# multiplefish/VPLines-SLAM

Hardware: AMD Instinct MI355X
Metric: sliding-window BA solves/sec (10 KF, 200 pts + 80 lines, 5 iters) (higher is better)
Workload: dtype f64

## Files before the change

### vplines-slam_amd/csrc/ba_common.h

```cpp
#pragma once
#include <hip/hip_runtime.h>
#include "ba_types.h"
#include "vpl_math.h"

namespace vpl {

#ifdef VPL_STAMPS
#define VPL_STAMP(B, w, i) do { if (threadIdx.x == 0) (B).dbg[(size_t)(w) * 64 + (i)] = (long long)__builtin_readcyclecounter(); } while (0)
#define VPL_IVAL(acc) long long acc = 0
#define VPL_IVAL_START(t) long long t = __builtin_readcyclecounter()
#define VPL_IVAL_ADD(acc, t) acc += __builtin_readcyclecounter() - (t)
#define VPL_IVAL_LAP(acc, t) do { const long long now_ = __builtin_readcyclecounter(); acc += now_ - (t); t = now_; } while (0)
#define VPL_IVAL_STORE(cond, dst, ...) do { long long* dst_ = (dst); if (dst_ && (cond)) { const long long v_[] = {__VA_ARGS__}; \
  for (int i_ = 0; i_ < (int)(sizeof(v_) / sizeof(v_[0])); ++i_) dst_[i_] = v_[i_]; } } while (0)
#else
#define VPL_STAMP(B, w, i) do {} while (0)
#define VPL_IVAL(acc) do {} while (0)
#define VPL_IVAL_START(t) do {} while (0)
#define VPL_IVAL_ADD(acc, t) do {} while (0)
#define VPL_IVAL_LAP(acc, t) do {} while (0)
#define VPL_IVAL_STORE(cond, dst, ...) do {} while (0)
#endif

__device__ __forceinline__ void count_active(const DevBatch& B, int k) {
  if (B.act && threadIdx.x == 0 && B.launch < ACT_SLOTS) atomicAdd(&B.act[4 * B.launch + k], 1);
}

__device__ __forceinline__ int ordered_window(const DevBatch& B) {
  const int w = B.ord_it == 0 ? (int)blockIdx.x : B.order[(size_t)(B.ord_it & 1) * B.nW + blockIdx.x];
  return __builtin_amdgcn_readfirstlane(w);
}

__device__ __forceinline__ double wave_sum(double v) {
#pragma unroll
  for (int o = 32; o > 0; o >>= 1) v += __shfl_xor(v, o, 64);
  return v;
}

template <int CTRL>
__device__ __forceinline__ double dpp_shr_f64(double v) {
  const int lo = __builtin_amdgcn_update_dpp(0, __double2loint(v), CTRL, 0xf, 0xf, true);
  const int hi = __builtin_amdgcn_update_dpp(0, __double2hiint(v), CTRL, 0xf, 0xf, true);
  return __hiloint2double(hi, lo);
}
__device__ __forceinline__ double row_sum16(double v) {
  v += dpp_shr_f64<0x111>(v);
  v += dpp_shr_f64<0x112>(v);
  v += dpp_shr_f64<0x114>(v);
  v += dpp_shr_f64<0x118>(v);
  return v;
}

__device__ __forceinline__ double wave_sum_dpp(double v) {
  v = row_sum16(v);
  double t = 0.0;
#pragma unroll
  for (int l = 15; l < 64; l += 16)
    t += __hiloint2double(__builtin_amdgcn_readlane(__double2hiint(v), l), __builtin_amdgcn_readlane(__double2loint(v), l));
  return t;
}

__device__ __forceinline__ double block_sum(double v, double* red) {
  const int lane = threadIdx.x & 63, wv = threadIdx.x >> 6, nw = (blockDim.x + 63) >> 6;
  v = wave_sum(v);
  __syncthreads();
  if (lane == 0) red[wv] = v;
  __syncthreads();
  if (threadIdx.x == 0) {
    double s = 0;
    for (int i = 0; i < nw; ++i) s += red[i];
    red[16] = s;
  }
  __syncthreads();
  return red[16];
}

__device__ __forceinline__ void lds_add(double* p, double v) { unsafeAtomicAdd(p, v); }

__host__ __device__ __forceinline__ int cam2vis(int c) {
  if (c >= 165) return 66 + (c - 165);
  int o = c % 15;
  return o < 6 ? 6 * (c / 15) + o : -1;
}

__device__ __forceinline__ void tri_decode(int idx, int& r, int& c) {
  int rr = (int)((sqrtf(8.0f * (float)idx + 1.0f) - 1.0f) * 0.5f);
  while ((rr + 1) * (rr + 2) / 2 <= idx) ++rr;
  while (rr * (rr + 1) / 2 > idx) --rr;
  r = rr;
  c = idx - rr * (rr + 1) / 2;
}

__device__ __forceinline__ PreInt load_preint(const DevPreint& d) {
  PreInt p;
  p.sum_dt = d.sum_dt;
  p.dp = V3{d.dp[0], d.dp[1], d.dp[2]};
  p.dv = V3{d.dv[0], d.dv[1], d.dv[2]};
  p.dq = Q4{d.dq[3], d.dq[0], d.dq[1], d.dq[2]};
  p.lba = V3{d.lba[0], d.lba[1], d.lba[2]};
  p.lbg = V3{d.lbg[0], d.lbg[1], d.lbg[2]};
#pragma unroll
  for (int k = 0; k < 9; ++k) {
    p.dp_dba.m[k] = d.dp_dba[k];
    p.dp_dbg.m[k] = d.dp_dbg[k];
    p.dq_dbg.m[k] = d.dq_dbg[k];
    p.dv_dba.m[k] = d.dv_dba[k];
    p.dv_dbg.m[k] = d.dv_dbg[k];
  }
  return p;
}

__device__ __forceinline__ void prior_block_dx(int kind, const double* x, const double* x0, double* dx) {
  if (kind == 1) {
#pragma unroll
    for (int k = 0; k < 9; ++k) dx[k] = x[k] - x0[k];
  } else {
    dx[0] = x[0] - x0[0]; dx[1] = x[1] - x0[1]; dx[2] = x[2] - x0[2];
    Q4 dq = qmul(qinv(qpose(x0)), qpose(x));
    double sgn = (dq.w >= 0) ? 2.0 : -2.0;
    dx[3] = sgn * dq.x; dx[4] = sgn * dq.y; dx[5] = sgn * dq.z;
  }
}

__device__ __forceinline__ double readlane_f64(double v, int srclane) {
  const int lo = __builtin_amdgcn_readlane(__double2loint(v), srclane);
  const int hi = __builtin_amdgcn_readlane(__double2hiint(v), srclane);
  return __hiloint2double(hi, lo);
}
template <int J>
__device__ __forceinline__ double swizzle_row_f64(double v) {
  const int lo = __builtin_amdgcn_mov_dpp(__double2loint(v), 0x150 + J, 0xf, 0xf, false);
  const int hi = __builtin_amdgcn_mov_dpp(__double2hiint(v), 0x150 + J, 0xf, 0xf, false);
  return __hiloint2double(hi, lo);
}

template <int J>
// ... 63 lines not shown
```

### vplines-slam_amd/csrc/ba_ctx.h

```cpp
#pragma once
#include <functional>
#include <map>
#include <string>

#include "vplines_ba.h"
#include "ba_types.h"
#include "ba_stage.h"
#include "ba_restore.h"

struct vpl_ctx {
  int device = 0;
  hipStream_t stream = nullptr;
  DevBatch B;
  std::vector<DevAlloc> allocs;
  bool guards = false;
  std::string err;
  int maxW = 0, maxP = 0, maxPO = 0, maxL = 0, maxLO = 0;
  int nW = 0;
  vpl_ba_options opt;
  bool upload_open = false;
  std::vector<int> h_nP, h_nL;
  std::vector<std::vector<int>> h_lmap;
  std::vector<int> h_mg_m;
  std::vector<int> h_mg_n;
  std::vector<int> h_mg_nb;
  std::vector<int> h_passthrough;
  std::vector<vpl_prior> h_pass_priors;
  bool any_second_new = false;
  int maxPriorN = 0;
  bool prior_resident = false;
  int prior_resident_nW = 0;
  std::vector<int> layout_key;
  bool layout_valid = false;
  bool force_general = false;
  bool schur_mostly_wide = false;
  bool schur_never_wide = false;
  bool schur_wide_all = false;
  bool step_fused = true;
  size_t marg_smem = 0;
  int marg_nmax = 0;
  bool marg_small = false;
  int prior_rule = VPL_PRIOR_PIVOTED_CHOLESKY;
  hipGraphExec_t graph_exec[3] = {nullptr, nullptr, nullptr};
  bool use_graph = true;
  int restore_pending = RESTORE_NONE;
  bool restore_fold = true;
  bool timing = false;
  std::map<std::string, std::pair<double, int>> ktimes;
  std::vector<std::pair<const char*, double>> ltimes;
  int* d_act = nullptr;
  std::vector<std::string> kname_store;
  bool leg_timing = false;
  hipEvent_t leg_ev[6] = {nullptr, nullptr, nullptr, nullptr, nullptr, nullptr};
  double odo_ms[3] = {0, 0, 0};
  std::function<int()> pending;
  Stage stage;
  size_t last_upload_bytes = 0;
  struct vpl_odo* odo = nullptr;
};

static void drop_graph(vpl_ctx* c) {
  for (hipGraphExec_t& g : c->graph_exec)
    if (g) { (void)hipGraphExecDestroy(g); g = nullptr; }
}

static int restore_states(vpl_ctx* c, int mode) {
  if (mode == RESTORE_NONE || c->nW < 1) return VPL_OK;
  const DevBatch& B = c->B;
  const size_t W = c->nW;
  HIPCHK(c, hipSetDevice(c->device));
  HIPCHK(c, hipMemcpyAsync(B.pose, B.pose_0, W * 77 * 8, hipMemcpyDeviceToDevice, c->stream));
  HIPCHK(c, hipMemcpyAsync(B.sb, B.sb_0, W * 99 * 8, hipMemcpyDeviceToDevice, c->stream));
  HIPCHK(c, hipMemcpyAsync(B.ex, B.ex_0, W * 7 * 8, hipMemcpyDeviceToDevice, c->stream));
  HIPCHK(c, hipMemcpyAsync(B.invd, B.invd_0, W * B.maxP * 8, hipMemcpyDeviceToDevice, c->stream));
  if (mode == RESTORE_LINES) HIPCHK(c, hipMemcpyAsync(B.plk, B.plk_0, W * B.maxL * 6 * 8, hipMemcpyDeviceToDevice, c->stream));
  return VPL_OK;
}
static int restore_event(vpl_ctx* c, RestoreEvent ev, int* prep = nullptr) {
  const RestoreStep s = restore_step(c->restore_pending, ev, c->restore_fold);
  c->restore_pending = s.pending;
  if (prep) *prep = s.prep;
  return restore_states(c, s.flush);
// ... 50 lines not shown
```

### vplines-slam_amd/csrc/ba_lin.h

```cpp
#pragma once
#include "ba_common.h"

namespace vpl {

typedef double v4d_lin __attribute__((ext_vector_type(4)));
constexpr int LIN_THREADS = 512;
constexpr int STG_LD = 17;
constexpr int LIN_STAGE = 8 * 32 * STG_LD;
constexpr int PRE_LDS = 62;
constexpr int LIN_HW = 720;
constexpr int PREP_NMAX = 112;
__host__ __device__ constexpr int lin_stage_doubles(int maxL) {
  const int ln = 8 * LIN_HW + 38 * maxL;
  const int pt = LIN_STAGE + 78 * 36 + NV;
  const int m = ln > pt ? ln : pt;
  return m > 4650 + 3570 ? m : 4650 + 3570;
}
constexpr int PREP_THREADS = 640;
inline size_t prep_smem(int max_prior_n) {
  const int ns = max_prior_n < PREP_NMAX ? max_prior_n : PREP_NMAX;
  return (size_t)((PREP_THREADS / 64) * 675 + ns * ns + ns + 84) * sizeof(double);
}
constexpr size_t PREP_SMEM = (size_t)((PREP_THREADS / 64) * 675 + PREP_NMAX * PREP_NMAX + PREP_NMAX + 84) * sizeof(double);

// ... 146 lines not shown
          acc = __builtin_amdgcn_mfma_f64_16x16x4f64(av, bv, acc, 0, 0, 0);
        }
        const double vals[4] = {acc.x, acc.y, acc.z, acc.w};
#pragma unroll
        for (int v = 0; v < 4; ++v) {
          const int r = 16 * ta + kk + 4 * v, c2 = cb;
          if (r < n && c2 < n && (ta != tb || r >= c2)) {
            H[(size_t)r * n + c2] = vals[v];
            H[(size_t)c2 * n + r] = vals[v];
          }
        }
      }
    } else
    for (int idx = tid; idx < n * n; idx += blockDim.x) {
      int a = idx / n, b = idx % n;
      double s = 0;
      for (int k = 0; k < n; ++k) s += Js[(size_t)k * n + a] * Js[(size_t)k * n + b];
      H[idx] = s;
    }
    for (int c2 = tid; c2 < n; c2 += blockDim.x) {
      double s = 0;
      if (fits) {
#pragma unroll 8
        for (int k = 0; k < n; ++k) s += Jl[k * n + c2] * r0s[k];
      } else {
        const double* r0g = B.pr_r0 + (size_t)w * MAXPN;
#pragma unroll 8
        for (int k = 0; k < n; ++k) s += J0[(size_t)k * n + c2] * r0g[k];
      }
      B.pr_g0[(size_t)w * MAXPN + c2] = s;
    }
    if (tid < B.pr_nb[w]) {
      int kind = B.pr_kind[(size_t)w * MAXPB + tid], fr = B.pr_frame[(size_t)w * MAXPB + tid];
      int idx = B.pr_idx[(size_t)w * MAXPB + tid];
      int base = kind == 0 ? 15 * fr : kind == 1 ? 15 * fr + 6 : 165;
      int ls = kind == 1 ? 9 : 6;
      for (int k = 0; k < ls; ++k) B.pr_map[(size_t)w * MAXPN + idx + k] = base + k;
    }
  }
  if (tid == 0) {
    TrState t;
    t.radius = 1e4; t.mu = 1e-8; t.x_cost = 0; t.cand_cost = 0; t.model_cost_change = 0; t.x_norm = 0;
    t.step_norm = 0; t.dogleg_step_norm = 0; t.alpha = 0; t.a1 = t.a2 = t.a3 = 0; t.initial_cost = 0;
    t.iter = 0; t.status = 0; t.reuse = 0; t.step_valid = 0; t.fresh_lin = 0; t.num_successful = 0; t.num_invalid = 0;
    t.pad = 0;
    B.tr[w] = t;
  }
}
__global__ __launch_bounds__(PREP_THREADS) void k_prep(DevBatch B, int nstage, int restore) {
  extern __shared__ double psm[];
  prep_body(B, blockIdx.x, psm, nstage, restore);
}

constexpr int HV_DOUBLES = 78 * 36;
constexpr int LIN_PART = 78 * 36 + 72 + 8;
__host__ __device__ __forceinline__ int hvi(int r, int c) {
  const int br = r / 6, bc = c / 6;
  return 36 * (br * (br + 1) / 2 + bc) + 6 * (r - 6 * br) + (c - 6 * bc);
}

inline void lin_asm_entry(int r, int c, int* out) {
  int hv = 0, im = 0;
  const int vr = cam2vis(r), vc = cam2vis(c);
  if (vr >= 0 && vc >= 0) hv = hvi(vr, vc) + 1;
  if (r < 165) {
    const int fr = r / 15, ar = r - 15 * fr, fc = c / 15, bc = c - 15 * fc;
    if (fc == fr) im = 120 * fr + ar * (ar + 1) / 2 + bc + 1;
    else if (fc == fr - 1) im = 11 * 120 + 225 * (fr - 1) + 15 * ar + bc + 1;
  }
  out[0] = hv | im << 16;
  out[1] = r | c << 8;
}


__device__ __forceinline__ double* lin_pt_stage(double* imuJ, int wvi) { return imuJ + wvi * (32 * STG_LD); }
__device__ __forceinline__ double* lin_Hv2(double* imuJ) { return imuJ + LIN_STAGE; }
__device__ __forceinline__ double* lin_ln_Hw(double* imuJ, int wvi) { return imuJ + wvi * LIN_HW; }
__device__ __forceinline__ double* lin_ln_acc(double* imuJ) { return imuJ + 8 * LIN_HW; }
__device__ __forceinline__ double* lin_imuH(double* imuJ) { return imuJ + 4650; }

struct PriorBlock {
  int kind = 0, fr = 0, idx = 0;
  double x0[9];
};
__device__ __forceinline__ void prior_block_request(const DevBatch& B, const int w, const int tid, const int nb, PriorBlock& b) {
  if (tid < nb) {
    b.kind = B.pr_kind[(size_t)w * MAXPB + tid]; b.fr = B.pr_frame[(size_t)w * MAXPB + tid]; b.idx = B.pr_idx[(size_t)w * MAXPB + tid];
#pragma unroll
    for (int k = 0; k < 9; ++k) b.x0[k] = B.pr_x0[((size_t)w * MAXPB + tid) * 9 + k];
  }
}
__device__ __forceinline__ void prior_block_dx_store(const PriorBlock& b, const int tid, const int nb, const double* xp, const double* xs,
                                                     double* prdx) {
  if (tid < nb) {
    const double* x = b.kind == 0 ? xp + 7 * b.fr : b.kind == 1 ? xs + 9 * b.fr : xp + 77;
    double dx[9];
    prior_block_dx(b.kind, x, b.x0, dx);
    const int ls = b.kind == 1 ? 9 : 6;
    for (int k = 0; k < ls; ++k) prdx[b.idx + k] = dx[k];
  }
}
constexpr int LIN_PJ = 6;
struct PriorRegs {
  int n = 0, nb = 0;
  PriorBlock blk;
  int pmap = -1;
  double j0[LIN_PJ], hv[LIN_PJ], r0 = 0.0, g0 = 0.0;
};
constexpr int LIN_ASM_PER_THREAD = (NCP + LIN_THREADS - 1) / LIN_THREADS;

template <int ROLE>
__device__ __forceinline__ void lin_stage(const DevBatch& B, const int w, double* sm, double* xp, double* xs, double* pacc, const int PST, double* plds,
                                             int* invmap, int* tick, PriorRegs& P) {
  constexpr bool DO_PTS = ROLE != 2, DO_REST = ROLE != 1;
  const int tid = threadIdx.x, T = LIN_THREADS;
  for (int i = tid; i < HV_DOUBLES + NV; i += T) sm[i] = 0.0;
  if (DO_PTS) for (int i = tid; i < 14 * PST; i += T) pacc[i] = 0.0;
  for (int i = tid; i < 84; i += T) xp[i] = i < 77 ? B.pose[(size_t)w * 77 + i] : B.ex[(size_t)w * 7 + (i - 77)];
  if (DO_REST) {
    for (int i = tid; i < 99; i += T) xs[i] = B.sb[(size_t)w * 99 + i];
    for (int i = tid; i < 10 * PRE_LDS; i += T) {
      const int f = i / PRE_LDS;
      plds[i] = ((const double*)&B.pre[(size_t)w * NF + f + 1])[i - PRE_LDS * f];
    }
  }
  for (int i = tid; i < NC; i += T) invmap[i] = -1;
  if (tid < 5) tick[tid] = 0;
  P.n = DO_REST ? B.pr_n[w] : 0; P.nb = P.n > 0 ? B.pr_nb[w] : 0;
  const int n = P.n;
  const int prow = tid >> 3, psub = tid & 7;
  prior_block_request(B, w, tid, P.nb, P.blk);
  if (tid < n) P.pmap = B.pr_map[(size_t)w * MAXPN + tid];
  {
    const double* J0 = B.pr_J0 + (size_t)w * B.prS;
    const double* Hp = B.pr_H + (size_t)w * B.prS;
#pragma unroll
    for (int q = 0; q < LIN_PJ; ++q) {
      const int c = psub + 8 * q;
      const bool in = prow < n && c < n;
      P.j0[q] = in ? J0[(size_t)prow * n + c] : 0.0;
      P.hv[q] = in ? Hp[(size_t)prow * n + c] : 0.0;
    }
    if (prow < n && psub == 0) { P.r0 = B.pr_r0[(size_t)w * MAXPN + prow]; P.g0 = B.pr_g0[(size_t)w * MAXPN + prow]; }
  }
}

__device__ __forceinline__ void lin_prior(const DevBatch& B, const int w, const double* xp, const double* xs, double* prdx, double* prr, double* prg,
                                             double* prH, const int PRH_N, int* invmap, const PriorRegs& P, double& cost) {
  const int tid = threadIdx.x, T = LIN_THREADS;
  const int n = P.n;
  const int prow = tid >> 3, psub = tid & 7;
  double r0r = P.r0, g0r = P.g0;
  if (n > 0) {
    prior_block_dx_store(P.blk, tid, P.nb, xp, xs, prdx);
    if (tid < n) invmap[P.pmap] = tid;
    for (int i = tid + T; i < n; i += T) invmap[B.pr_map[(size_t)w * MAXPN + i]] = i;
    __syncthreads();
    const double* J0 = B.pr_J0 + (size_t)w * B.prS;
    const double* Hp = B.pr_H + (size_t)w * B.prS;
    for (int r = prow; r < n; r += T >> 3) {
      const bool first = r == prow;
      double s = 0, sg = 0;
// ... 116 lines not shown
        Hv[hvi(66 + a, 6 * f + c2)] += v;
      } else {
        gv[6 * f + (q - 57)] += v;
      }
    } else if (e < 714) {
      int a, c2;
      tri_decode(e - 693, a, c2);
      Hv[hvi(66 + a, 66 + c2)] += v;
    } else {
      gv[66 + (e - 714)] += v;
    }
  }
}

template <int MODE>
__device__ __forceinline__ void lin_imu_raw(const DevBatch& B, const int w, const double* xp, const double* xs, const double* plds, double* imuJ, double* imur,
                                               int* imuact, double (&sa)[2][4]) {
  constexpr bool MARG = MODE != 0;
  constexpr bool PRIOR_ONLY = MODE == 2;
  const int tid = threadIdx.x, T = LIN_THREADS, lane = tid & 63;
  for (int i = tid; i < 4650; i += T) imuJ[i] = 0.0;
#pragma unroll
  for (int q = 0; q < 2; ++q) {
    const int f = (tid >> 6) + 8 * q;
    const double* S = B.pre[(size_t)w * NF + (f < 10 ? f : 0) + 1].sqrt_info;
#pragma unroll
    for (int ks = 0; ks < 4; ++ks) {
      const int k = 4 * ks + (lane >> 4), i = lane & 15;
      sa[q][ks] = (f < 10 && i < 15 && k < 15 && k >= i) ? S[i * 15 + k] : 0.0;
    }
  }
  __syncthreads();
  if ((tid & 63) < 10 && tid < 128) {
    const int f = tid & 63, j = f + 1;
    const DevPreint& dp = *(const DevPreint*)(plds + PRE_LDS * f);
    bool act = MARG ? (j == 1 && dp.sum_dt < 10.0) : !(dp.sum_dt > 10.0);
    if (PRIOR_ONLY) act = false;
    if (tid < 64) imuact[f] = act ? 1 : 0;
    if (act) {
      PreInt p = load_preint(dp);
      if (tid < 64) {
        imu_residual_raw(p, xp + 7 * (j - 1), xs + 9 * (j - 1), xp + 7 * j, xs + 9 * j, B.opt.g_norm, imur + 15 * f);
      } else {
        ImuJac JB = imu_jacobian_raw(p, xp + 7 * (j - 1), xs + 9 * (j - 1), xp + 7 * j, xs + 9 * j, B.opt.g_norm);
        imu_jac_dense(JB, imuJ + 450 * f);
      }
    }
  }
}
__device__ __forceinline__ void lin_asm_request(const DevBatch& B, int2 (&asmd)[LIN_ASM_PER_THREAD]) {
  const int tid = threadIdx.x, T = LIN_THREADS;
#pragma unroll
  for (int u = 0; u < LIN_ASM_PER_THREAD; ++u) {
    const int e = u * T + tid;
    asmd[u] = ((const int2*)B.asm_tab)[e < NCP ? e : 0];
  }
}
__device__ __forceinline__ void lin_imu_whiten(double* imuJ, double* imur, const int* imuact, const double (&sa)[2][4]) {
  const int tid = threadIdx.x, T = LIN_THREADS, lane = tid & 63;
  double* imuH = lin_imuH(imuJ);
  const int wvi = tid >> 6, m16 = lane & 15, kk = lane >> 4;
  v4d_lin cd[2] = {{0, 0, 0, 0}, {0, 0, 0, 0}};
  for (int i = tid; i < 120; i += T) imuH[i] = 0.0;
#pragma unroll
  for (int q = 0; q < 2; ++q) {
    const int f = wvi + 8 * q;
    if (f >= 10) break;
    double* J = imuJ + 450 * f;
    double* rr = imur + 15 * f;
    const bool on = imuact[f] != 0;
    v4d_lin jw[2] = {{0, 0, 0, 0}, {0, 0, 0, 0}};
#pragma unroll
    for (int ct = 0; ct < 2; ++ct) {
      const int c = 16 * ct + m16;
#pragma unroll
      for (int ks = 0; ks < 4; ++ks) {
        const int k = 4 * ks + kk;
        const double bv = k < 15 ? (c < 30 ? J[k * 30 + c] : (c == 30 ? rr[k] : 0.0)) : 0.0;
        jw[ct] = __builtin_amdgcn_mfma_f64_16x16x4f64(on ? sa[q][ks] : 0.0, bv, jw[ct], 0, 0, 0);
      }
    }
    __builtin_amdgcn_wave_barrier();
    if (on) {
#pragma unroll
      for (int ct = 0; ct < 2; ++ct) {
        const double vals[4] = {jw[ct].x, jw[ct].y, jw[ct].z, jw[ct].w};
        const int c = 16 * ct + m16;
#pragma unroll
        for (int v = 0; v < 4; ++v) {
          const int r = kk + 4 * v;
          if (r < 15) {
            if (c < 30) J[r * 30 + c] = vals[v];
            else if (c == 30) rr[r] = vals[v];
          }
        }
      }
    }
    __builtin_amdgcn_fence(__ATOMIC_RELEASE, "workgroup");
    __builtin_amdgcn_wave_barrier();
    __builtin_amdgcn_fence(__ATOMIC_ACQUIRE, "workgroup");
    v4d_lin c00 = {0, 0, 0, 0}, c10 = {0, 0, 0, 0}, c11 = {0, 0, 0, 0};
#pragma unroll
    for (int ks = 0; ks < 4; ++ks) {
      const int k = 4 * ks + kk;
      const double lo = k < 15 ? J[k * 30 + m16] : 0.0;
      const double hi = (k < 15 && m16 < 14) ? J[k * 30 + 16 + m16] : 0.0;
      c00 = __builtin_amdgcn_mfma_f64_16x16x4f64(lo, lo, c00, 0, 0, 0);
      c10 = __builtin_amdgcn_mfma_f64_16x16x4f64(hi, lo, c10, 0, 0, 0);
// ... 6 lines not shown
      for (int v = 0; v < 4; ++v) {
        const int i0 = kk + 4 * v, j0 = m16;
        if (i0 < 15 && j0 < 15) keep[v] = v00[v];
        const int i1 = 16 + kk + 4 * v;
        if (i1 < 30) {
          if (j0 < 15) imuH[11 * 120 + 225 * f + 15 * (i1 - 15) + j0] = v10[v];
          else imuH[120 * (f + 1) + (i1 - 15) * (i1 - 14) / 2 + 0] = v10[v];
          const int j1 = 16 + m16;
          if (j1 < 30 && j1 <= i1) imuH[120 * (f + 1) + (i1 - 15) * (i1 - 14) / 2 + (j1 - 15)] = v11[v];
        }
        if (i0 == 15) {
          if (j0 < 15) imuH[11 * 120 + 225 * f + j0] = v00[v];
          else imuH[120 * (f + 1)] = v00[v];
        }
      }
      cd[q] = v4d_lin{keep[0], keep[1], keep[2], keep[3]};
    }
  }
  __syncthreads();
#pragma unroll
  for (int q = 0; q < 2; ++q) {
    const int f = wvi + 8 * q;
    if (f >= 10) break;
    const double keep[4] = {cd[q].x, cd[q].y, cd[q].z, cd[q].w};
#pragma unroll
    for (int v = 0; v < 4; ++v) {
      const int i0 = kk + 4 * v, j0 = m16;
      if (i0 < 15 && j0 <= i0) imuH[120 * f + i0 * (i0 + 1) / 2 + j0] += keep[v];
    }
  }
}
__device__ __forceinline__ void lin_imu_cost(const double* imur, const int* imuact, double& cost) {
  const int tid = threadIdx.x;
  if (tid < 10 && imuact[tid]) {
    double s = 0;
    for (int k = 0; k < 15; ++k) s += imur[15 * tid + k] * imur[15 * tid + k];
    cost += 0.5 * s;
  }
}

__device__ __forceinline__ void lin_handover_in(const DevBatch& B, const int w, double* sm, double& cost) {
  const int tid = threadIdx.x, T = LIN_THREADS;
  if (tid == 0) {
    while (__hip_atomic_load(&B.lin_flag[w], __ATOMIC_RELAXED, __HIP_MEMORY_SCOPE_AGENT) != 1) __builtin_amdgcn_s_sleep(32);
    __hip_atomic_store(&B.lin_flag[w], 0, __ATOMIC_RELAXED, __HIP_MEMORY_SCOPE_AGENT);
  }
  __syncthreads();
  const double* part = B.lin_part + (size_t)w * LIN_PART;
  for (int i = tid; i < HV_DOUBLES + NV; i += T) sm[i] += __hip_atomic_load(&part[i], __ATOMIC_RELAXED, __HIP_MEMORY_SCOPE_AGENT);
  if (tid == 0) cost += __hip_atomic_load(&part[HV_DOUBLES + NV], __ATOMIC_RELAXED, __HIP_MEMORY_SCOPE_AGENT);
  __syncthreads();
}

__device__ __forceinline__ void lin_assemble(const DevBatch& B, const int w, const double* Hv, const double* gv, double* imuJ, const double* imur,
                                                const double* prg, const double* prH, const int PRH_N, const int* invmap,
                                                const int* imuact, const int n, const bool ex_free,
                                                const int2 (&asmd)[LIN_ASM_PER_THREAD]) {
  const int tid = threadIdx.x, T = LIN_THREADS;
  const double* const imuH = lin_imuH(imuJ);
  double* Hout = B.Hcc + (size_t)w * NCP;
  const double* pH = B.pr_H + (size_t)w * B.prS;
  VPL_STAMP(B, w, 26);
  const bool prior_lds = n > 0 && n <= PRH_N;
  {
#pragma unroll
    for (int u = 0; u < LIN_ASM_PER_THREAD; ++u) {
      const int e = u * T + tid;
      if (e >= NCP) continue;
      const int hv = asmd[u].x & 0xffff, im = asmd[u].x >> 16, r = asmd[u].y & 255, c = asmd[u].y >> 8;
      const double vh = Hv[hv ? hv - 1 : 0], vi = imuH[im ? im - 1 : 0];
      const int ir = prior_lds ? invmap[r] : -1, ic = prior_lds ? invmap[c] : -1;
      const bool hp = ir >= 0 && ic >= 0;
      const int hi_ = ic > ir ? ic : ir, lo_ = ic > ir ? ir : ic;
      const double vp = prH[hp ? hi_ * (hi_ + 1) / 2 + lo_ : 0];
      double v = hv ? vh : 0.0;
      v += im ? vi : 0.0;
      v += hp ? vp : 0.0;
      if (!ex_free && r >= 165) v = 0.0;
      Hout[e] = v;
    }
  }
  VPL_STAMP(B, w, 27);
  if (n > PRH_N) {
    __syncthreads();
    const int np = n * (n + 1) / 2;
    for (int base = 0; base < np; base += 4 * T) {
      double ph[4];
      int tr_[4], tc_[4];
#pragma unroll
      for (int u = 0; u < 4; ++u) {
        const int e = base + u * T + tid;
        ph[u] = 0.0; tr_[u] = -1; tc_[u] = 0;
        if (e < np) {
          int i, j;
          tri_decode(e, i, j);
          ph[u] = pH[(size_t)i * n + j];
          const int ri = B.pr_map[(size_t)w * MAXPN + i], rj = B.pr_map[(size_t)w * MAXPN + j];
          tr_[u] = ri > rj ? ri : rj;
          tc_[u] = ri > rj ? rj : ri;
        }
      }
#pragma unroll
      for (int u = 0; u < 4; ++u)
        if (tr_[u] >= 0 && (ex_free || tr_[u] < 165)) Hout[(size_t)tr_[u] * (tr_[u] + 1) / 2 + tc_[u]] += ph[u];
    }
  }
  for (int r = tid; r < NC; r += T) {
    double v = 0.0;
    const int vr = cam2vis(r);
    if (vr >= 0) v += gv[vr];
    if (r < 165) {
      const int fr = r / 15;
      if (fr >= 1 && imuact[fr - 1]) {
        const double* J = imuJ + 450 * (fr - 1);
        const double* rr = imur + 15 * (fr - 1);
        const int a = r - 15 * (fr - 1);
        double s = 0;
#pragma unroll
        for (int k = 0; k < 15; ++k) s += J[k * 30 + a] * rr[k];
        v += s;
      }
      if (fr < 10 && imuact[fr]) {
        const double* J = imuJ + 450 * fr;
        const double* rr = imur + 15 * fr;
        const int a = r - 15 * fr;
        double s = 0;
#pragma unroll
        for (int k = 0; k < 15; ++k) s += J[k * 30 + a] * rr[k];
        v += s;
      }
    }
    if (n > 0 && invmap[r] >= 0) v += prg[invmap[r]];
// ... 437 lines not shown
```

### vplines-slam_amd/csrc/ba_upload.h

```cpp
#pragma once
#include "ba_ctx.h"
#include "ba_odo.h"
#include "ba_pack.h"
#include "host_common.h"

static void to_dev_preint(const vpl_preintegration& p, DevPreint& d) {
  d.sum_dt = p.sum_dt;
  for (int k = 0; k < 3; ++k) { d.dp[k] = p.delta_p[k]; d.dv[k] = p.delta_v[k]; d.lba[k] = p.linearized_ba[k]; d.lbg[k] = p.linearized_bg[k]; }
  for (int k = 0; k < 4; ++k) d.dq[k] = p.delta_q[k];
  auto blk = [&](double* o, int r0, int c0) {
    for (int i = 0; i < 3; ++i)
      for (int j = 0; j < 3; ++j) o[3 * i + j] = p.jacobian[(r0 + i) * 15 + c0 + j];
  };
  blk(d.dp_dba, 0, 9); blk(d.dp_dbg, 0, 12); blk(d.dq_dbg, 3, 12); blk(d.dv_dba, 6, 9); blk(d.dv_dbg, 6, 12);
  std::memcpy(d.cov, p.covariance, sizeof(d.cov));
  std::memset(d.sqrt_info, 0, sizeof(d.sqrt_info));
}

struct UploadArena {
  Span<double> pose, sb, ex, invd, plk, pt_obs, ln_obs, fail_ref, orth, pr_x0, pr_r0;
  Span<int> nP, nL, pt_start, pt_nobs, pt_off, ln_start, ln_nobs, ln_off, ln_tri, pu_cnt, pu_cnt0, sk_tab, sk_wave, path, nLO, lo_ln,
      ll_tab, ll_np, ps_list, ps_cnt, orth_in, pr_n, pr_nb, pr_kind, pr_frame, pr_idx, mg_n, mg_nb, mg_kind, mg_frame, mg_idx, mg_cam, mg_m;
  Span<DevPreint> pre;
  std::vector<Span<double>> J0;
// ... 424 lines not shown
  B.opt.marginalization_flag = opt->marginalization_flag;
  B.opt.remove_line_outliers = opt->remove_line_outliers;
  B.opt.sqrt_info_point = opt->focal_length / 1.5;
  B.opt.sqrt_info_line = opt->line_factor;
  B.opt.sqrt_info_vp = opt->vp_factor;
  B.opt.g_norm = opt->g_norm;
  B.opt.huber_delta = opt->huber_delta;
  const size_t W = nW;
  std::vector<HostTab> ctab;
  if (chained && (rc = read_resident_priors(c, W, ctab))) return rc;
  const bool dev_prior = chained || odo;
  if (odo) {
    ctab.assign(W, HostTab());
    for (size_t w = 0; w < W; ++w)
      if (odo->tab && odo->has[w]) ctab[w] = odo->tab[w];
  }
  c->h_mg_m.assign(W, 0);
  c->maxPriorN = 0;
  c->h_passthrough.assign(W, -1);
  c->h_pass_priors.clear();
  c->any_second_new = false;
  c->h_nP.assign(W, 0);
  c->h_nL.assign(W, 0);
  c->h_lmap.resize(W);
  if ((rc = batch_strides(c, W, win, opt, dev_prior ? ctab.data() : nullptr))) return rc;
  const bool same_layout = layout_unchanged(c, W, win, all_lines);
  Stage& SG = c->stage;
  HIPCHK(c, SG.reserve(upload_bound(B, W, win, same_layout, dev_prior, odo)));
  UploadArena A;
  take_upload(SG, A, B, W, win, dev_prior, odo);
  std::unique_ptr<int[]> lane(new int[W * B.maxPR * 1024]), sub(new int[W * B.maxPR * 512]);
  long schur_wide_w = 0, schur_total_w = 0;
  for (size_t w = 0; w < W; ++w) {
    const HostTab* T = dev_prior ? &ctab[w] : nullptr;
    if ((rc = pack_tracks(c, A, w, win[w], all_lines))) return rc;
    if (odo) pack_gather(c, A, w, win[w], *odo);
    else pack_values(c, A, w, win[w]);
    if (!same_layout &&
        (rc = build_layout(c, A, w, win[w], &lane[w * B.maxPR * 1024], &sub[w * B.maxPR * 512], &schur_wide_w, &schur_total_w)))
      return rc;
    if ((rc = pack_prior(c, A, w, win[w], T))) return rc;
    if ((rc = keep_blocks(c, A, w, win[w], T))) return rc;
  }
  if ((rc = choose_marg(c, A.mg_n, W))) return rc;
  if (!same_layout) pack_units(SG, A, W, B.maxPR, lane.get(), sub.get());
  std::memcpy(A.mg_m.p, c->h_mg_m.data(), W * 4);
  c->h_mg_n.assign(A.mg_n.begin(), A.mg_n.end());
  c->h_mg_nb.assign(A.mg_nb.begin(), A.mg_nb.end());
  if (odo)
    for (size_t w = 0; w < W; ++w)
      A.odo_marg[w] = (opt->marginalization_flag != VPL_MARGIN_NONE && c->h_passthrough[w] < 0) ? 1 + A.mg_nb[w] : 0;
  if (!same_layout) c->schur_mostly_wide = schur_total_w > 0 && 20 * schur_wide_w > 7 * schur_total_w;
  if (c->force_general) std::fill(A.path.begin(), A.path.end(), 1);
  if (SG.overflow) return fail(c, VPL_E_CAPACITY, "internal: staging arena bound too small");
  stage_upload(SG, A, B, W, same_layout, dev_prior, odo);
  if (chained && (rc = hand_over_priors(c, ctab, prev_prS))) return rc;
  HIPCHK(c, stage_run(c->stage, c->stream, true, &c->last_upload_bytes));
  if (odo) {
    hipLaunchKernelGGL(k_odo_gather, dim3(nW), dim3(ODO_THREADS), 0, c->stream, B, odo->store, (const int*)odo->d_psrc, (const int*)odo->d_lsrc);
    if (odo->tab) hipLaunchKernelGGL(k_odo_prior_load, dim3(nW), dim3(ODO_THREADS), 0, c->stream, B, odo->prior, (const int*)odo->d_has);
    HIPCHK(c, hipGetLastError());
  }
  if (c->leg_timing) HIPCHK(c, hipEventRecord(c->leg_ev[1], c->stream));
  HIPCHK(c, hipStreamSynchronize(c->stream));
  c->layout_valid = true;
  return VPL_OK;
}
static int upload_impl(vpl_ctx* c, int nW, const vpl_window* win, const vpl_ba_options* opt, bool all_lines, bool chained = false,
                       const OdoSrc* odo = nullptr) {
  const int rc = upload_body(c, nW, win, opt, all_lines, chained, odo);
  if (c) {
    if (rc != VPL_OK && c->upload_open) { c->nW = 0; c->prior_resident = false; }
    c->upload_open = false;
  }
  return rc;
}
```

### vplines-slam_amd/csrc/vplines_ba.hip

```cpp
#include <hip/hip_runtime.h>

#include <algorithm>
#include <chrono>
#include <memory>
#include <cstdlib>
#include <cstring>
#include <string>
#include <vector>

#include "vplines_ba.h"
#include "ba_types.h"
#include "ba_lin.h"
#include "ba_pack.h"
#include "ba_solve.h"
#include "ba_step.h"
#include "ba_marg.h"
#include "ba_prior_eig.h"
#include "ba_lineopt.h"
#include "ba_factors.h"
#include "ba_odo.h"
#include "odo_tracks.h"
#include "host_common.h"

using namespace vpl;
// ... 72 lines not shown
  c->maxW = max_windows;
  c->maxP = max_points > 0 ? (max_points + 1) & ~1 : 2;
  c->maxPO = max_point_obs > 0 ? max_point_obs : 1;
  c->maxL = max_lines > 0 ? max_lines : 1;
  c->maxLO = max_line_obs > 0 ? max_line_obs : 1;
  if (!solve_layout_fits(c->maxP, c->maxL)) return VPL_E_CAPACITY;
  if (solve_smem(c->maxP, c->maxL) > 159 * 1024) return VPL_E_CAPACITY;
  DevBatch& B = c->B;
  std::memset(&B, 0, sizeof(B));
  B.maxP = c->maxP; B.maxPO = c->maxPO; B.maxL = c->maxL; B.maxLO = c->maxLO;
  B.nfull = NC + B.maxP + 4 * B.maxL;
  {
    int ncu = 0;
    if (hipDeviceGetAttribute(&ncu, hipDeviceAttributeMultiprocessorCount, device) != hipSuccess || ncu <= 0) ncu = 256;
    if (const char* sv = std::getenv("VPL_BA_LIN_SPLIT")) ncu = std::atoi(sv) ? 1 << 30 : 0;
    B.ncu = ncu;
  }
  B.maxPR = max_point_unit_rounds(B.maxP, B.maxPO);
  B.maxKS = max_schur_ksteps(B.maxP, B.maxL);
  B.llSlots = line_lane_slots(B.maxL);
  const size_t W = max_windows;
  hipError_t e = hipSuccess;
#define AL(ptr, n) if (e == hipSuccess) e = dalloc(c, &B.ptr, (size_t)(n))
  AL(pose, W * 77); AL(sb, W * 99); AL(ex, W * 7); AL(invd, W * B.maxP); AL(orth, W * B.maxL * 4);
  AL(pose_c, W * 77); AL(sb_c, W * 99); AL(ex_c, W * 7); AL(invd_c, W * B.maxP); AL(orth_c, W * B.maxL * 4); AL(lw, W * B.maxL * 6); AL(lw_c, W * B.maxL * 6);
  AL(lin_part, W * LIN_PART); AL(lin_pcost, W); AL(lin_flag, W);
  AL(pose_0, W * 77); AL(sb_0, W * 99); AL(ex_0, W * 7); AL(invd_0, W * B.maxP); AL(plk_0, W * B.maxL * 6);
  AL(plk, W * B.maxL * 6); AL(gauge, W * 4); AL(fail_ref, W * 13); AL(orth_in, W);
  AL(nP, W); AL(nL, W);
  AL(pt_start, W * B.maxP); AL(pt_nobs, W * B.maxP); AL(pt_off, W * B.maxP); AL(pt_obs, W * B.maxPO * 3);
  AL(ps_list, W * B.maxP); AL(ps_cnt, W * (NF + 1)); AL(pu_lane, W * B.maxPR * 1024); AL(pu_sub, W * B.maxPR * 512); AL(pu_cnt, W); AL(pu_cnt0, W);
  AL(ln_start, W * B.maxL); AL(ln_nobs, W * B.maxL); AL(ln_off, W * B.maxL); AL(ln_obs, W * B.maxLO * 8);
  AL(nLO, W); AL(lo_ln, W * B.maxLO);
  AL(ll_tab, W * B.llSlots * 2); AL(ll_np, W);
  AL(pre, W * NF);
  AL(pr_n, W); AL(pr_nb, W); AL(pr_kind, W * MAXPB); AL(pr_frame, W * MAXPB); AL(pr_idx, W * MAXPB);
  AL(pr_x0, W * MAXPB * 9); AL(pr_J0, W * MAXPN * MAXPN); AL(pr_r0, W * MAXPN); AL(pr_H, W * MAXPN * MAXPN); AL(pr_g0, W * MAXPN);
  AL(pr_map, W * MAXPN);
  AL(Hcc, W * NCP); AL(gc, W * NC); AL(asm_tab, 2 * NCP); AL(Hpp, W * B.maxP); AL(gp, W * B.maxP); AL(Wp, W * B.maxP * NV);
  AL(Hll, W * B.maxL * 16); AL(gl, W * B.maxL * 4); AL(Wl, W * B.maxL * 4 * NV); AL(lchol, W * B.maxL * 10);
  AL(tr, W);
  AL(scale, W * B.nfull); AL(diag, W * B.nfull); AL(grad, W * B.nfull); AL(gn, W * B.nfull);
  AL(mg_n, W); AL(mg_nb, W); AL(mg_kind, W * MAXPB); AL(mg_frame, W * MAXPB); AL(mg_idx, W * MAXPB);
  AL(mg_cam, W * MAXPB); AL(mg_x0, W * MAXPB * 9); AL(mg_J0, W * MAXKEEP * MAXKEEP); AL(mg_r0, W * MAXKEEP);
  AL(mg_A, W * MAXKEEP * MAXKEEP); AL(mg_b, W * MAXKEEP); AL(mg_m, W); AL(dbg, W * 64); AL(ln_removed, W * B.maxL); AL(ln_tri, W * B.maxL);
  if (e == hipSuccess) e = dalloc(c, &c->d_act, (size_t)ACT_SLOTS * 4);
  AL(order, 2 * W); AL(ord_cnt, 4);
  AL(sk_tab, W * B.maxKS * 4); AL(sk_wave, W * 8 * SK_WSTRIDE); AL(sacc, W * SACC_N); AL(nz_tab, NZ_N); AL(ycs, W * 176); AL(sx, W * 8); AL(path, W);
#undef AL
  if (e != hipSuccess) return VPL_E_HIP;
  if (lin_smem_base(c->maxP, c->maxL) > LIN_LDS_BUDGET) return VPL_E_CAPACITY;
  B.prhN = lin_prh_n(c->maxP, c->maxL);
  {
    std::vector<int> tab(2 * NCP);
    for (int r = 0, e2 = 0; r < NC; ++r)
      for (int cc = 0; cc <= r; ++cc, ++e2) lin_asm_entry(r, cc, &tab[2 * e2]);
    if (hipMemcpy(B.asm_tab, tab.data(), tab.size() * sizeof(int), hipMemcpyHostToDevice) != hipSuccess) return VPL_E_HIP;
  }
  {
    std::vector<int> nz;
    for (int r = 0; r < NC; ++r)
      for (int cc = 0; cc <= r; ++cc) {
        const bool vis = cam2vis(r) >= 0 && cam2vis(cc) >= 0;
        const int fr = r < 165 ? r / 15 : -1, fc = cc < 165 ? cc / 15 : -1;
        const bool band = fr >= 0 && fc >= 0 && (fr == fc || fr == fc + 1);
        const bool sb0 = cc >= 6 && cc < 15 && cam2vis(r) >= 0;
        if (vis || band || sb0) nz.push_back(tri(r, cc) | r << 14 | cc << 22);
      }
    if ((int)nz.size() != NZ_N || hipMemcpy(B.nz_tab, nz.data(), nz.size() * sizeof(int), hipMemcpyHostToDevice) != hipSuccess) return VPL_E_HIP;
  }
  static size_t lin_max = 0, solve_max = 0, schur_max = 0, back_max = 0, step_max = 0;
  lin_max = std::max(lin_max, lin_smem(c->maxP, c->maxL));
  solve_max = std::max(solve_max, solve_smem(c->maxP, c->maxL));
  schur_max = std::max(schur_max, schur_smem(c->maxP, c->maxL));
  back_max = std::max(back_max, back_smem(c->maxP, c->maxL));
  step_max = std::max(step_max, step_smem(c->maxP, c->maxL));
  if (schur_max > 159 * 1024 || back_max > 159 * 1024) return VPL_E_CAPACITY;
  const std::pair<const void*, size_t> lds[] = {
      {(const void*)k_lin2, lin_max}, {(const void*)k_lin<1>, lin_max}, {(const void*)k_lin<2>, lin_max},
      {(const void*)k_solve, solve_max}, {(const void*)k_schur<3>, schur_max}, {(const void*)k_schur<5>, schur_max},
      {(const void*)k_schur_mixed, schur_max}, {(const void*)k_chol, chol_smem()}, {(const void*)k_back, back_max},
      {(const void*)k_step<3, false>, step_max}, {(const void*)k_step<3, true>, step_max}, {(const void*)k_step<5, false>, step_max},
      {(const void*)k_prep, PREP_SMEM}, {(const void*)k_marg<MARG_THREADS>, MARG_LDS_MAX}, {(const void*)k_marg<256>, MARG_LDS_SMALL},
      {(const void*)k_prior_eigen, prior_eig_layout(MAXKEEP).bytes}, {(const void*)k_init_align, init_lds_bytes(INIT_NMAX)}};
  for (const auto& k : lds)
    if (hipFuncSetAttribute(k.first, hipFuncAttributeMaxDynamicSharedMemorySize, (int)k.second) != hipSuccess) return VPL_E_HIP;
  vpl_ba_default_options(&c->opt);
  if (const char* gv = std::getenv("VPL_BA_GRAPH")) c->use_graph = std::atoi(gv) != 0;
  if (const char* gv = std::getenv("VPL_BA_GENERAL")) c->force_general = std::atoi(gv) != 0;
  if (const char* gv = std::getenv("VPL_BA_STEP_FUSED")) c->step_fused = std::atoi(gv) != 0;
  if (const char* gv = std::getenv("VPL_BA_RESET_FOLD")) c->restore_fold = std::atoi(gv) != 0;
  if (const char* gv = std::getenv("VPL_BA_SCHUR_WIDE")) { c->schur_wide_all = std::atoi(gv) > 0; c->schur_never_wide = std::atoi(gv) < 0; }
  return VPL_OK;
}

int vpl_ctx_create(vpl_ctx** out, int device, int max_windows, int max_points, int max_point_obs, int max_lines,
                   int max_line_obs) {
  if (!out || max_windows < 1 || max_points < 0 || max_lines < 0) return VPL_E_INVALID;
  int ndev = 0;
  if (hipGetDeviceCount(&ndev) != hipSuccess || ndev == 0 || device >= ndev) return VPL_E_NODEVICE;
  if (hipSetDevice(device) != hipSuccess) return VPL_E_NODEVICE;
  vpl_ctx* c = new vpl_ctx();
  const int rc = ctx_init(c, device, max_windows, max_points, max_point_obs, max_lines, max_line_obs);
  if (rc != VPL_OK) {
    free_arrays(c);
    delete c;
    return rc;
  }
  *out = c;
  return VPL_OK;
}

void vpl_ctx_destroy(vpl_ctx* c) {
  if (!c) return;
  (void)hipSetDevice(c->device);
  (void)hipDeviceSynchronize();
  (void)restore_event(c, RESTORE_EV_DESTROY);
  drop_graph(c);
  free_arrays(c);
  c->stage.release();
  for (hipEvent_t& e : c->leg_ev) if (e) (void)hipEventDestroy(e);
  delete c;
// ... 986 lines not shown
```

Measured before the change: 268,900.

## Assemble only structurally nonzero Hcc entries, handling complement on general path

Reorders the Hessian assembly table so entries in the known sparsity pattern come first. The linearization kernel now writes only those entries by default, and writes the complement only for windows on the general path. To keep the skipped entries valid, Hcc is zeroed with a memset on upload when the previous batch used the general path. This cuts per-thread table loads and stores in the assembly step, but it relies on untouched entries staying zero and adds an occasional device memset.

After: 274,900, median of 6. 2.2% higher.

```diff
diff --git a/vplines-slam_amd/csrc/ba_asm_pattern.h b/vplines-slam_amd/csrc/ba_asm_pattern.h
--- /dev/null
+++ b/vplines-slam_amd/csrc/ba_asm_pattern.h
@@ -0,0 +1,63 @@
+#pragma once
+#include <vector>
+
+#include "ba_types.h"
+
+namespace vpl {
+
+#ifdef __HIPCC__
+#define VPL_ASM_HD __host__ __device__ __forceinline__
+#else
+#define VPL_ASM_HD inline
+#endif
+
+VPL_ASM_HD int cam2vis(int c) {
+  if (c >= 165) return 66 + (c - 165);
+  int o = c % 15;
+  return o < 6 ? 6 * (c / 15) + o : -1;
+}
+
+constexpr int HV_DOUBLES = 78 * 36;
+VPL_ASM_HD int hvi(int r, int c) {
+  const int br = r / 6, bc = c / 6;
+  return 36 * (br * (br + 1) / 2 + bc) + 6 * (r - 6 * br) + (c - 6 * bc);
+}
+
+inline void lin_asm_entry(int r, int c, int* out) {
+  int hv = 0, im = 0;
+  const int vr = cam2vis(r), vc = cam2vis(c);
+  if (vr >= 0 && vc >= 0) hv = hvi(vr, vc) + 1;
+  if (r < 165) {
+    const int fr = r / 15, ar = r - 15 * fr, fc = c / 15, bc = c - 15 * fc;
+    if (fc == fr) im = 120 * fr + ar * (ar + 1) / 2 + bc + 1;
+    else if (fc == fr - 1) im = 11 * 120 + 225 * (fr - 1) + 15 * ar + bc + 1;
+  }
+  out[0] = hv | im << 16;
+  out[1] = r | c << 8 | tri(r, c) << 16;
+}
+
+inline bool asm_in_pattern(int r, int c) {
+  const bool vis = cam2vis(r) >= 0 && cam2vis(c) >= 0;
+  const int fr = r < 165 ? r / 15 : -1, fc = c < 165 ? c / 15 : -1;
+  const bool band = fr >= 0 && fc >= 0 && (fr == fc || fr == fc + 1);
+  const bool sb0 = c >= 6 && c < 15 && cam2vis(r) >= 0;
+  return vis || band || sb0;
+}
+constexpr int NZ_C = NCP - NZ_N;
+
+inline void asm_build_tables(std::vector<int>& nz, std::vector<int>& asm_tab) {
+  nz.clear();
+  std::vector<int> pat, comp;
+  for (int r = 0; r < NC; ++r)
+    for (int c = 0; c <= r; ++c) {
+      int d[2];
+      lin_asm_entry(r, c, d);
+      std::vector<int>& t = asm_in_pattern(r, c) ? pat : comp;
+      t.push_back(d[0]); t.push_back(d[1]);
+      if (asm_in_pattern(r, c)) nz.push_back(tri(r, c) | r << 14 | c << 22);
+    }
+  asm_tab = pat;
+  asm_tab.insert(asm_tab.end(), comp.begin(), comp.end());
+}
+
+}
diff --git a/vplines-slam_amd/csrc/ba_common.h b/vplines-slam_amd/csrc/ba_common.h
--- a/vplines-slam_amd/csrc/ba_common.h
+++ b/vplines-slam_amd/csrc/ba_common.h
@@ -1,6 +1,7 @@
 #pragma once
 #include <hip/hip_runtime.h>
 #include "ba_types.h"
+#include "ba_asm_pattern.h"
 #include "vpl_math.h"
 
 namespace vpl {
@@ -77,11 +78,6 @@
 
 __device__ __forceinline__ void lds_add(double* p, double v) { unsafeAtomicAdd(p, v); }
 
-__host__ __device__ __forceinline__ int cam2vis(int c) {
-  if (c >= 165) return 66 + (c - 165);
-  int o = c % 15;
-  return o < 6 ? 6 * (c / 15) + o : -1;
-}
 
 __device__ __forceinline__ void tri_decode(int idx, int& r, int& c) {
   int rr = (int)((sqrtf(8.0f * (float)idx + 1.0f) - 1.0f) * 0.5f);
diff --git a/vplines-slam_amd/csrc/ba_ctx.h b/vplines-slam_amd/csrc/ba_ctx.h
--- a/vplines-slam_amd/csrc/ba_ctx.h
+++ b/vplines-slam_amd/csrc/ba_ctx.h
@@ -28,6 +28,7 @@
   std::vector<vpl_prior> h_pass_priors;
   bool any_second_new = false;
   int maxPriorN = 0;
+  bool hcc_general = false;
   bool prior_resident = false;
   int prior_resident_nW = 0;
   std::vector<int> layout_key;
diff --git a/vplines-slam_amd/csrc/ba_lin.h b/vplines-slam_amd/csrc/ba_lin.h
--- a/vplines-slam_amd/csrc/ba_lin.h
+++ b/vplines-slam_amd/csrc/ba_lin.h
@@ -222,25 +222,7 @@
   prep_body(B, blockIdx.x, psm, nstage, restore);
 }
 
-constexpr int HV_DOUBLES = 78 * 36;
 constexpr int LIN_PART = 78 * 36 + 72 + 8;
-__host__ __device__ __forceinline__ int hvi(int r, int c) {
-  const int br = r / 6, bc = c / 6;
-  return 36 * (br * (br + 1) / 2 + bc) + 6 * (r - 6 * br) + (c - 6 * bc);
-}
-
-inline void lin_asm_entry(int r, int c, int* out) {
-  int hv = 0, im = 0;
-  const int vr = cam2vis(r), vc = cam2vis(c);
-  if (vr >= 0 && vc >= 0) hv = hvi(vr, vc) + 1;
-  if (r < 165) {
-    const int fr = r / 15, ar = r - 15 * fr, fc = c / 15, bc = c - 15 * fc;
-    if (fc == fr) im = 120 * fr + ar * (ar + 1) / 2 + bc + 1;
-    else if (fc == fr - 1) im = 11 * 120 + 225 * (fr - 1) + 15 * ar + bc + 1;
-  }
-  out[0] = hv | im << 16;
-  out[1] = r | c << 8;
-}
 
 
 __device__ __forceinline__ double* lin_pt_stage(double* imuJ, int wvi) { return imuJ + wvi * (32 * STG_LD); }
@@ -277,7 +259,7 @@
   int pmap = -1;
   double j0[LIN_PJ], hv[LIN_PJ], r0 = 0.0, g0 = 0.0;
 };
-constexpr int LIN_ASM_PER_THREAD = (NCP + LIN_THREADS - 1) / LIN_THREADS;
+constexpr int LIN_ASM_PER_THREAD = (NZ_N + LIN_THREADS - 1) / LIN_THREADS;
 
 template <int ROLE>
 __device__ __forceinline__ void lin_stage(const DevBatch& B, const int w, double* sm, double* xp, double* xs, double* pacc, const int PST, double* plds,
@@ -500,8 +482,8 @@
   const int tid = threadIdx.x, T = LIN_THREADS;
 #pragma unroll
   for (int u = 0; u < LIN_ASM_PER_THREAD; ++u) {
-    const int e = u * T + tid;
-    asmd[u] = ((const int2*)B.asm_tab)[e < NCP ? e : 0];
+    const int i = u * T + tid;
+    asmd[u] = ((const int2*)B.asm_tab)[i < NZ_N ? i : 0];
   }
 }
 __device__ __forceinline__ void lin_imu_whiten(double* imuJ, double* imur, const int* imuact, const double (&sa)[2][4]) {
@@ -614,6 +596,20 @@
   __syncthreads();
 }
 
+__device__ __forceinline__ void lin_asm_store(const int2 d, const double* Hv, const double* imuH, const double* prH, const int* invmap,
+                                                 const bool prior_lds, const bool ex_free, double* Hout) {
+  const int hv = d.x & 0xffff, im = d.x >> 16, r = d.y & 255, c = (d.y >> 8) & 255, e = d.y >> 16;
+  const double vh = Hv[hv ? hv - 1 : 0], vi = imuH[im ? im - 1 : 0];
+  const int ir = prior_lds ? invmap[r] : -1, ic = prior_lds ? invmap[c] : -1;
+  const bool hp = ir >= 0 && ic >= 0;
+  const int hi_ = ic > ir ? ic : ir, lo_ = ic > ir ? ir : ic;
+  const double vp = prH[hp ? hi_ * (hi_ + 1) / 2 + lo_ : 0];
+  double v = hv ? vh : 0.0;
+  v += im ? vi : 0.0;
+  v += hp ? vp : 0.0;
+  if (!ex_free && r >= 165) v = 0.0;
+  Hout[e] = v;
+}
 __device__ __forceinline__ void lin_assemble(const DevBatch& B, const int w, const double* Hv, const double* gv, double* imuJ, const double* imur,
                                                 const double* prg, const double* prH, const int PRH_N, const int* invmap,
                                                 const int* imuact, const int n, const bool ex_free,
@@ -627,19 +623,22 @@
   {
 #pragma unroll
     for (int u = 0; u < LIN_ASM_PER_THREAD; ++u) {
-      const int e = u * T + tid;
-      if (e >= NCP) continue;
-      const int hv = asmd[u].x & 0xffff, im = asmd[u].x >> 16, r = asmd[u].y & 255, c = asmd[u].y >> 8;
-      const double vh = Hv[hv ? hv - 1 : 0], vi = imuH[im ? im - 1 : 0];
-      const int ir = prior_lds ? invmap[r] : -1, ic = prior_lds ? invmap[c] : -1;
-      const bool hp = ir >= 0 && ic >= 0;
-      const int hi_ = ic > ir ? ic : ir, lo_ = ic > ir ? ir : ic;
-      const double vp = prH[hp ? hi_ * (hi_ + 1) / 2 + lo_ : 0];
-      double v = hv ? vh : 0.0;
-      v += im ? vi : 0.0;
-      v += hp ? vp : 0.0;
-      if (!ex_free && r >= 165) v = 0.0;
-      Hout[e] = v;
+      if (u * T + tid >= NZ_N) continue;
+      lin_asm_store(asmd[u], Hv, imuH, prH, invmap, prior_lds, ex_free, Hout);
+    }
+  }
+  if (B.path[w] == 1) {
+    const int2* const ctab = (const int2*)B.asm_tab + NZ_N;
+    for (int base = 0; base < NZ_C; base += 4 * T) {
+      int2 d[4];
+#pragma unroll
+      for (int u = 0; u < 4; ++u) {
+        const int i = base + u * T + tid;
+        d[u] = ctab[i < NZ_C ? i : 0];
+      }
+#pragma unroll
+      for (int u = 0; u < 4; ++u)
+        if (base + u * T + tid < NZ_C) lin_asm_store(d[u], Hv, imuH, prH, invmap, prior_lds, ex_free, Hout);
     }
   }
   VPL_STAMP(B, w, 27);
diff --git a/vplines-slam_amd/csrc/ba_upload.h b/vplines-slam_amd/csrc/ba_upload.h
--- a/vplines-slam_amd/csrc/ba_upload.h
+++ b/vplines-slam_amd/csrc/ba_upload.h
@@ -500,6 +500,8 @@
       A.odo_marg[w] = (opt->marginalization_flag != VPL_MARGIN_NONE && c->h_passthrough[w] < 0) ? 1 + A.mg_nb[w] : 0;
   if (!same_layout) c->schur_mostly_wide = schur_total_w > 0 && 20 * schur_wide_w > 7 * schur_total_w;
   if (c->force_general) std::fill(A.path.begin(), A.path.end(), 1);
+  if (c->hcc_general) HIPCHK(c, hipMemsetAsync(B.Hcc, 0, (size_t)c->maxW * NCP * sizeof(double), c->stream));
+  c->hcc_general = std::any_of(A.path.begin(), A.path.end(), [](int p) { return p != 0; });
   if (SG.overflow) return fail(c, VPL_E_CAPACITY, "internal: staging arena bound too small");
   stage_upload(SG, A, B, W, same_layout, dev_prior, odo);
   if (chained && (rc = hand_over_priors(c, ctab, prev_prS))) return rc;
diff --git a/vplines-slam_amd/csrc/vplines_ba.hip b/vplines-slam_amd/csrc/vplines_ba.hip
--- a/vplines-slam_amd/csrc/vplines_ba.hip
+++ b/vplines-slam_amd/csrc/vplines_ba.hip
@@ -148,22 +148,11 @@
   if (lin_smem_base(c->maxP, c->maxL) > LIN_LDS_BUDGET) return VPL_E_CAPACITY;
   B.prhN = lin_prh_n(c->maxP, c->maxL);
   {
-    std::vector<int> tab(2 * NCP);
-    for (int r = 0, e2 = 0; r < NC; ++r)
-      for (int cc = 0; cc <= r; ++cc, ++e2) lin_asm_entry(r, cc, &tab[2 * e2]);
+    std::vector<int> nz, tab;
+    asm_build_tables(nz, tab);
+    if ((int)nz.size() != NZ_N || (int)tab.size() != 2 * NCP) return VPL_E_HIP;
     if (hipMemcpy(B.asm_tab, tab.data(), tab.size() * sizeof(int), hipMemcpyHostToDevice) != hipSuccess) return VPL_E_HIP;
-  }
-  {
-    std::vector<int> nz;
-    for (int r = 0; r < NC; ++r)
-      for (int cc = 0; cc <= r; ++cc) {
-        const bool vis = cam2vis(r) >= 0 && cam2vis(cc) >= 0;
-        const int fr = r < 165 ? r / 15 : -1, fc = cc < 165 ? cc / 15 : -1;
-        const bool band = fr >= 0 && fc >= 0 && (fr == fc || fr == fc + 1);
-        const bool sb0 = cc >= 6 && cc < 15 && cam2vis(r) >= 0;
-        if (vis || band || sb0) nz.push_back(tri(r, cc) | r << 14 | cc << 22);
-      }
-    if ((int)nz.size() != NZ_N || hipMemcpy(B.nz_tab, nz.data(), nz.size() * sizeof(int), hipMemcpyHostToDevice) != hipSuccess) return VPL_E_HIP;
+    if (hipMemcpy(B.nz_tab, nz.data(), nz.size() * sizeof(int), hipMemcpyHostToDevice) != hipSuccess) return VPL_E_HIP;
   }
   static size_t lin_max = 0, solve_max = 0, schur_max = 0, back_max = 0, step_max = 0;
   lin_max = std::max(lin_max, lin_smem(c->maxP, c->maxL));
```
